# zalo/TetSim

Hardware: AMD Instinct MI355X
Metric: tet_solves_per_sec (higher is better)
Workload: dtype f32; 1 GPU; Kuhn-6 cube lattice 55x55x55 cells (998250 tets, 175616 particles), polar-decomposition Jacobi, 20 substeps/frame, dt=1/1200 s; solver=polar_jacobi, arithmetic=fast, formulation=reference (rest shape carried from substep to substep, 148 B/tet), tets=998250, particles=175616, parallelism=single GPU

## Files before the change

### tetsim_amd/csrc/pj_blocked.hip

```cpp
#define TETSIM_FAST 1
#include <cstdio>
#include <algorithm>
#include <cstdlib>
#include <type_traits>
#include <vector>

#include "collide.h"
#include "dev_common.h"
#include "dev_store.h"
#include "host_prep.h"
#include "pj_lab.h"

namespace tetsim {
namespace {

#include "pj_math.inc"
#include "pj_blocked_lab.inc"


__device__ __forceinline__ uint32_t xcd_tile(uint32_t b, uint32_t tiles_per_xcd) { return (b & 7u) * tiles_per_xcd + (b >> 3); }

struct VertexOut { f3 p, vel, pred; };
__device__ __forceinline__ VertexOut pjb_vertex_update(f3 acc, float wsum, f3 prev, const DevParams& P, uint32_t v) {
    const float rw = __builtin_amdgcn_rcpf(wsum);
    f3 p = F3(acc.x * rw, acc.y * rw, acc.z * rw);
    const bool grabbed = static_cast<int32_t>(v) == P.grab_local || static_cast<int32_t>(v) == P.grab_local2;
    if (grabbed) p = F3(P.grab[0], P.grab[1], P.grab[2]);
    p.x = fminf(fmaxf(p.x, P.lo[0]), P.hi[0]);
    p.y = fminf(fmaxf(p.y, P.lo[1]), P.hi[1]);
    p.z = fminf(fmaxf(p.z, P.lo[2]), P.hi[2]);
    if (p.y < 0.0f) {
        p.y = 0.0f;
        const float Fx = prev.x - p.x, Fz = prev.z - p.z;
        const float fr = fminf(1.0f, P.dt * P.friction);
        p.x = fmaf(Fx, fr, p.x);
        p.z = fmaf(Fz, fr, p.z);
    }
    if (P.n_colliders != 0u && !grabbed) collide_f32<true>(p.x, p.y, p.z, prev.x, prev.y, prev.z, P);
    const float dt = P.dt;
    const float rdt = __builtin_amdgcn_rcpf(dt);
    VertexOut o;
    o.p = p;
    const float gx = dt * 0.0f, gy = dt * P.gravity, gz = dt * 0.0f;
    o.vel = F3(fmaf(rdt, p.x - prev.x, gx), fmaf(rdt, p.y - prev.y, gy), fmaf(rdt, p.z - prev.z, gz));
    o.pred = F3(fmaf(dt, o.vel.x, p.x), fmaf(dt, o.vel.y, p.y), fmaf(dt, o.vel.z, p.z));
    return o;
}

constexpr uint32_t kTile = kBlockTile;

__device__ __forceinline__ f3 lean_fourth_corner(const f3 r[4]) {
    return F3(-((r[0].x + r[1].x) + r[2].x), -((r[0].y + r[1].y) + r[2].y), -((r[0].z + r[1].z) + r[2].z));
}
struct PJHaloWait { const PJPeerSync* w; const uint32_t* vflag; uint32_t* error; uint32_t timeout_ms; const float4* ghosts; };
constexpr int kModeCarried = 0, kModeConstantRest = 1, kModeLeanState = 2;
inline int blk_mode(const PJBlk& d) { return pjb_mode(d); }
struct PJPoll { uint32_t block, want; uint32_t* error; uint32_t timeout_ms; };
template <int kMode, bool kFused, bool kAlt = false, bool kHaloWait = false, bool kPoll = false>
__device__ __forceinline__ void pjb_tet_body(const PJBlk& d, uint32_t tile_first, uint32_t tile_count, uint32_t tiles_per_xcd TETSIM_DBG_PARAM,
                                             [[maybe_unused]] const PJHaloWait* hw = nullptr, const uint32_t stamp = 0u, [[maybe_unused]] const PJPoll* poll = nullptr) {
    __shared__ float4 s_pos[kTile];
    __shared__ float s_gx[4 * kTile];
    __shared__ float s_gy[4 * kTile];
    __shared__ float s_gz[4 * kTile];
    __shared__ uint2 s_ent[kTile];

    constexpr bool kLean = kMode == kModeConstantRest;
    uint32_t block_index = blockIdx.x;
    if constexpr (kPoll) block_index = poll->block;
    const uint32_t rel = xcd_tile(block_index, tiles_per_xcd);
    if (rel >= tile_count) return;
    const uint32_t b = tile_first + rel;
    const uint32_t tid = threadIdx.x;
    TETSIM_LAB_TILE_BEGIN();
    const uint32_t t0 = d.blk_tet_off[b], ntb = d.blk_tet_off[b + 1] - t0;
    const uint32_t v0 = d.blk_vert_off[b], nu = d.blk_vert_off[b + 1] - v0;

    const bool has_slot = tid < nu, has_tet = tid < ntb;
    const uint32_t slot = v0 + (has_slot ? tid : 0u), e = t0 + (has_tet ? tid : 0u);
    const uint32_t vid = static_cast<uint32_t>(d.blk_verts[slot]);
    const uint32_t range = has_slot ? d.lc_range[slot] : 0u;
    uint32_t src[8];
    uint32_t src8 = 0xffffffffu;
    [[maybe_unused]] uint32_t maxsrc = 0;
    if constexpr (kFused) {
        maxsrc = d.blk_maxsrc[b];
        const uint32_t* col = d.slot_src + slot;
#pragma unroll
        for (uint32_t j = 0; j < 8u; j++) src[j] = (j < maxsrc) ? col[static_cast<size_t>(j) * d.ns_pad] : 0xffffffffu;
        if (maxsrc > 8u) src8 = col[8ull * d.ns_pad];
    }
    const uchar4 li = d.tet_lidx[e];
    auto rec4 = [](const float4* a, uint32_t i) { if constexpr (kPoll) return load_coherent(a, i); else return a[i]; };
    float4 ra = make_float4(0.0f, 0.0f, 0.0f, 0.0f), rb = ra, rc = ra, q_old = make_float4(0.0f, 0.0f, 0.0f, 1.0f);
    auto load_record = [&]() {
        ra = rec4(d.rest_a, e); rb = rec4(d.rest_b, e);
        if constexpr (kMode == kModeLeanState) { if constexpr (kPoll) rc.x = load_coherent1(d.rest_c1, e); else rc.x = d.rest_c1[e]; }
        else { rc = rec4(d.rest_c, e); q_old = rec4(d.quat, e); }
    };
    bool record_late = false;
    if constexpr (kPoll) record_late = poll->want != 0u;
    if (!record_late) load_record();
    const float V = d.vol[e];
    const uint2 ent_row = d.lc_ent[e];
    float4 pos_stage;
    if constexpr (kFused) {
        f3 g[8];
#pragma unroll
        for (uint32_t j = 0; j < 8u; j++) {
            const float4 t = d.partial_prev[src[j] == 0xffffffffu ? 0u : src[j]];
            g[j] = src[j] == 0xffffffffu ? F3(0.0f, 0.0f, 0.0f) : xyz(t);
        }
        const float4 t8 = d.partial_prev[src8 == 0xffffffffu ? 0u : src8];
        const float4 prev4 = d.fin_in[vid];
        const float wsum = d.wsum[vid];
        f3 acc = F3(0.0f, 0.0f, 0.0f);
#pragma unroll
        for (uint32_t j = 0; j < 8u; j++) { acc.x += g[j].x; acc.y += g[j].y; acc.z += g[j].z; }
        if (src8 != 0xffffffffu) { acc.x += t8.x; acc.y += t8.y; acc.z += t8.z; }
        if (maxsrc > 9u) {
            const uint32_t* col = d.slot_src + slot;
            for (uint32_t j = 9u; j < maxsrc; j++) {
                const uint32_t sj = col[static_cast<size_t>(j) * d.ns_pad];
                const float4 tj = d.partial_prev[sj == 0xffffffffu ? 0u : sj];
                if (sj != 0xffffffffu) { acc.x += tj.x; acc.y += tj.y; acc.z += tj.z; }
            }
        }
        const VertexOut o = pjb_vertex_update(acc, wsum, xyz(prev4), *d.params, vid);
        pos_stage = make_float4(o.pred.x, o.pred.y, o.pred.z, 0.0f);
        if (has_slot && ((range >> 15) & 1u)) {
            store_wt(d.fin_out, vid, make_float4(o.p.x, o.p.y, o.p.z, 0.0f));
            if (d.vel) store_wt(d.vel, vid, make_float4(o.vel.x, o.vel.y, o.vel.z, 0.0f));
        }
    } else if constexpr (kHaloWait) {
        if (tid < 64u) {
            const PJPeerSync& w = *hw->w;
            const uint32_t* word = tid == 0u ? hw->vflag : (tid <= w.n_wait ? w.wait[tid - 1u] : nullptr);
            bool pending = word != nullptr;
            const long long t0 = wall_clock64(), limit = 100000ll * hw->timeout_ms;
            while (true) {
                if (pending) pending = __hip_atomic_load(word, __ATOMIC_RELAXED, __HIP_MEMORY_SCOPE_SYSTEM) == 0u;
                if (__builtin_amdgcn_ballot_w64(pending) == 0ull) break;
                __builtin_amdgcn_s_sleep(16);
                if (limit && wall_clock64() - t0 > limit) { if (tid == 0) __hip_atomic_store(hw->error, 1u, __ATOMIC_RELAXED, __HIP_MEMORY_SCOPE_SYSTEM); break; }
            }
            if (w.delay_us && w.n_wait) { const long long d0 = wall_clock64(); while (wall_clock64() - d0 < 100ll * w.delay_us) __builtin_amdgcn_s_sleep(8); }
        }
        __syncthreads();
        const bool ghost = vid >= d.nv_owned;
        const float4 own = load_coherent(d.pos_pred, ghost ? 0u : vid), gh = load_coherent(hw->ghosts, ghost ? vid - d.nv_owned : 0u);
        pos_stage = ghost ? gh : own;
    } else if constexpr (kAlt) {
        const uint32_t g = vid - d.nv_owned;
        const float4* src = vid >= d.nv_owned ? (g < d.n_ghost1 ? d.ghost_alt + g : d.ghost2 + (g - d.n_ghost1)) : d.pos_pred + vid;
        pos_stage = *src;
    } else if constexpr (kPoll) {
        pos_stage = load_coherent(d.pos_pred, vid);
        if (poll->want != 0u) {
            bool pend = has_slot && __float_as_uint(pos_stage.w) != poll->want;
            if (__builtin_amdgcn_ballot_w64(pend) != 0ull) {
                const long long t0 = wall_clock64(), limit = 100000ll * poll->timeout_ms;
                do {
                    __builtin_amdgcn_s_sleep(TETSIM_POLL_SLEEP);
                    asm volatile("" ::: "memory");
                    if (pend) { pos_stage = load_coherent(d.pos_pred, vid); pend = __float_as_uint(pos_stage.w) != poll->want; }
                    if (limit && pend && wall_clock64() - t0 > limit) { __hip_atomic_store(poll->error, 1u, __ATOMIC_RELAXED, __HIP_MEMORY_SCOPE_SYSTEM); pend = false; }
                } while (__builtin_amdgcn_ballot_w64(pend) != 0ull);
            }
            __syncthreads();
            load_record();
        }
    } else {
        pos_stage = d.pos_pred[vid];
    }
    if (has_slot) s_pos[tid] = pos_stage;
    if (has_tet) s_ent[tid] = ent_row;
    TETSIM_STAMP(1);
    __builtin_amdgcn_s_waitcnt(0x0F70);
    __syncthreads();
    TETSIM_STAMP(2);

    if (has_tet) {
        f3 cur[4], rest[4], goal[4];
        cur[0] = xyz(s_pos[li.x]); cur[1] = xyz(s_pos[li.y]); cur[2] = xyz(s_pos[li.z]); cur[3] = xyz(s_pos[li.w]);
        rest[0] = F3(ra.x, ra.y, ra.z); rest[1] = F3(ra.w, rb.x, rb.y);
        rest[2] = F3(rb.z, rb.w, rc.x); rest[3] = F3(rc.y, rc.z, rc.w);
        if constexpr (kMode == kModeLeanState) rest[3] = lean_fourth_corner(rest);
        float4 q_new;
        f3 cc;
        TETSIM_LAB_SOLVE_TET(cur, rest, q_old, q_new, goal, cc);
        TETSIM_STAMP(3);
        const f3 vcc = cc * V;
#pragma unroll
        for (int k = 0; k < 4; k++) {
            s_gx[k * kTile + tid] = fmaf(goal[k].x, V, vcc.x);
            s_gy[k * kTile + tid] = fmaf(goal[k].y, V, vcc.y);
            s_gz[k * kTile + tid] = fmaf(goal[k].z, V, vcc.z);
        }
        if constexpr (kMode != kModeLeanState) store_wt(d.quat, e, q_new);
        if (!kLean && TETSIM_DBG_STORE_REST) {
            store_wt(d.rest_a, e, make_float4(goal[0].x, goal[0].y, goal[0].z, goal[1].x));
            store_wt(d.rest_b, e, make_float4(goal[1].y, goal[1].z, goal[2].x, goal[2].y));
            if constexpr (kMode == kModeLeanState) store_wt1(d.rest_c1, e, goal[2].z);
            else store_wt(d.rest_c, e, make_float4(goal[2].z, goal[3].x, goal[3].y, goal[3].z));
        }
    }
    TETSIM_STAMP(4);
    if constexpr (kPoll) __builtin_amdgcn_s_waitcnt(0x0F70);
    __syncthreads();
    TETSIM_STAMP(5);

    if (tid < nu) {
        const uint32_t first = range & 0x7ffu, last = range >> 16;
        const uint16_t* ent = reinterpret_cast<const uint16_t*>(s_ent);
        auto plane = [](const float* base, uint32_t byte_off) { return *reinterpret_cast<const float*>(reinterpret_cast<const char*>(base) + byte_off); };
        float4 acc = make_float4(0.0f, 0.0f, 0.0f, 0.0f);
        uint32_t i = first;
        for (; i + 4u <= last; i += 4u) {
            uint32_t o[4];
            float gx[4], gy[4], gz[4];
#pragma unroll
            for (uint32_t j = 0; j < 4u; j++) o[j] = static_cast<uint32_t>(ent[i + j]) << 2;
#pragma unroll
            for (uint32_t j = 0; j < 4u; j++) { gx[j] = plane(s_gx, o[j]); gy[j] = plane(s_gy, o[j]); gz[j] = plane(s_gz, o[j]); }
#pragma unroll
            for (uint32_t j = 0; j < 4u; j++) { acc.x += gx[j]; acc.y += gy[j]; acc.z += gz[j]; }
        }
        for (; i < last; i++) {
            const uint32_t o = static_cast<uint32_t>(ent[i]) << 2;
            acc.x += plane(s_gx, o); acc.y += plane(s_gy, o); acc.z += plane(s_gz, o);
        }
        acc.w = __uint_as_float(stamp);
        store_wt(d.partial, v0 + tid, acc);
    }
    TETSIM_STAMP(6);
}

__global__ __launch_bounds__(kTile, 2) void pjb_tet_kernel(PJBlk d, uint32_t tile_first, uint32_t tile_count,
                                                        uint32_t tiles_per_xcd TETSIM_DBG_PARAM) {
    pjb_tet_body<kModeCarried, false>(d, tile_first, tile_count, tiles_per_xcd TETSIM_DBG_ARG);
}
__global__ __launch_bounds__(kTile, 2) void pjb_tet_kernel_constant_rest(PJBlk d, uint32_t tile_first, uint32_t tile_count,
                                                                      uint32_t tiles_per_xcd TETSIM_DBG_PARAM) {
    pjb_tet_body<kModeConstantRest, false>(d, tile_first, tile_count, tiles_per_xcd TETSIM_DBG_ARG);
}
__global__ __launch_bounds__(kTile, 2) void pjb_tet_kernel_lean(PJBlk d, uint32_t tile_first, uint32_t tile_count,
                                                             uint32_t tiles_per_xcd TETSIM_DBG_PARAM) {
    pjb_tet_body<kModeLeanState, false>(d, tile_first, tile_count, tiles_per_xcd TETSIM_DBG_ARG);
}
__device__ __forceinline__ void clear_then_raise(uint32_t* clear, uint32_t* sig) {
    if (blockIdx.x == 0 && threadIdx.x == 0) {
        if (clear) __hip_atomic_store(clear, 0u, __ATOMIC_RELAXED, __HIP_MEMORY_SCOPE_AGENT);
        if (sig) __hip_atomic_store(sig, 1u, __ATOMIC_RELEASE, __HIP_MEMORY_SCOPE_AGENT);
    }
}
struct TetRaise { uint32_t* sig; uint32_t* clear; };
struct TetAlt { uint32_t unused; };
struct TetHwait { PJPeerSync w; const uint32_t* vflag; uint32_t* error; uint32_t timeout_ms; const float4* ghosts; };
struct TetFused { uint32_t unused; };
template <int kMode, class Extra>
__global__ __launch_bounds__(kTile, 2) void pjb_tet_kernel_x(PJBlk d, uint32_t tile_first, uint32_t tile_count, uint32_t tiles_per_xcd, Extra x TETSIM_DBG_PARAM) {
    if constexpr (std::is_same_v<Extra, TetRaise>) {
        clear_then_raise(x.clear, x.sig);
        pjb_tet_body<kMode, false>(d, tile_first, tile_count, tiles_per_xcd TETSIM_DBG_ARG);
    } else if constexpr (std::is_same_v<Extra, TetAlt>) {
        pjb_tet_body<kMode, false, true>(d, tile_first, tile_count, tiles_per_xcd TETSIM_DBG_ARG);
    } else if constexpr (std::is_same_v<Extra, TetHwait>) {
        if (blockIdx.x == 0 && threadIdx.x < x.w.n_raise) __hip_atomic_store(x.w.raise[threadIdx.x], 1u, __ATOMIC_RELEASE, __HIP_MEMORY_SCOPE_SYSTEM);
        const PJHaloWait hw = {&x.w, x.vflag, x.error, x.timeout_ms, x.ghosts};
        pjb_tet_body<kMode, false, false, true>(d, tile_first, tile_count, tiles_per_xcd TETSIM_DBG_ARG, &hw);
    } else {
        pjb_tet_body<kMode, true>(d, tile_first, tile_count, tiles_per_xcd TETSIM_DBG_ARG);
    }
}
template <class Extra>
void launch_tet_x(hipStream_t s, const PJBlk& d, uint32_t tile_first, uint32_t tile_count, const Extra& x, hipEvent_t e0 = nullptr, hipEvent_t e1 = nullptr) {
    if (tile_count == 0) return;
    const uint32_t per_xcd = (tile_count + 7u) / 8u;
    const int mode = blk_mode(d);
    auto* kernel = mode == kModeConstantRest ? pjb_tet_kernel_x<kModeConstantRest, Extra> : mode == kModeLeanState ? pjb_tet_kernel_x<kModeLeanState, Extra> : pjb_tet_kernel_x<kModeCarried, Extra>;
    if (e0) hipExtLaunchKernelGGL(kernel, dim3(per_xcd * 8u), dim3(kTile), 0, s, e0, e1, 0, d, tile_first, tile_count, per_xcd, x TETSIM_DBG_LAUNCH);
    else hipLaunchKernelGGL(kernel, dim3(per_xcd * 8u), dim3(kTile), 0, s, d, tile_first, tile_count, per_xcd, x TETSIM_DBG_LAUNCH);
}

constexpr int kFrameIters = TETSIM_LAB_FRAME_ITERS;
template <int kMode, bool kLocal>
__device__ __forceinline__ void pjb_frame_body(const PJBlk& d, const DevParams& P, const uint32_t n, const int32_t* const block_tile, float4* const pbuf0, float4* const pbuf1,
                                               uint32_t* const err, const uint32_t timeout_ms) {
    __shared__ float4 s_pos[kTile];
    __shared__ float s_gx[4 * kTile];
    __shared__ float s_gy[4 * kTile];
    __shared__ float s_gz[4 * kTile];
    __shared__ uint2 s_ent[kTile];

    constexpr bool kLean = kMode == kModeConstantRest;
    const int32_t bt = block_tile[blockIdx.x];
    if (bt < 0) return;
    const uint32_t b = static_cast<uint32_t>(bt);
    const uint32_t tid = threadIdx.x;
    TETSIM_LAB_FRAME_BEGIN();
    const uint32_t t0 = d.blk_tet_off[b], ntb = d.blk_tet_off[b + 1] - t0;
    const uint32_t v0 = d.blk_vert_off[b], nu = d.blk_vert_off[b + 1] - v0;
    const bool has_slot = tid < nu, has_tet = tid < ntb;
    const uint32_t slot = v0 + (has_slot ? tid : 0u), e = t0 + (has_tet ? tid : 0u);
    const uint32_t vid = static_cast<uint32_t>(d.blk_verts[slot]);
    const uint32_t range = has_slot ? d.lc_range[slot] : 0u;
    const uint32_t maxsrc = d.blk_maxsrc[b];
    uint32_t src[9];
    {
        const uint32_t* col = d.slot_src + slot;
#pragma unroll
        for (uint32_t j = 0; j < 9u; j++) src[j] = (has_slot && j < maxsrc) ? col[static_cast<size_t>(j) * d.ns_pad] : 0xffffffffu;
    }
    const uchar4 li = d.tet_lidx[e];
    const float4 ra = d.rest_a[e], rb = d.rest_b[e];
    float4 rc = make_float4(0.0f, 0.0f, 0.0f, 0.0f), q = make_float4(0.0f, 0.0f, 0.0f, 1.0f);
    if constexpr (kMode == kModeLeanState) rc.x = d.rest_c1[e];
    else { rc = d.rest_c[e]; q = d.quat[e]; }
    const float V = d.vol[e];
    s_ent[tid] = has_tet ? d.lc_ent[e] : make_uint2(0u, 0u);
    f3 rest[4];
    rest[0] = F3(ra.x, ra.y, ra.z); rest[1] = F3(ra.w, rb.x, rb.y);
    rest[2] = F3(rb.z, rb.w, rc.x); rest[3] = F3(rc.y, rc.z, rc.w);
    f3 prev = xyz(d.pos_final[vid]);
    const float wsum = d.wsum[vid];
    f3 stage = xyz(d.pos_pred[vid]);
    const uint32_t epoch = d.epoch ? d.epoch : P.epoch;
    const uint32_t first = range & 0x7ffu, last = range >> 16;
    const bool owner = has_slot && ((range >> 15) & 1u);
    float4* const pbuf[2] = {pbuf0, pbuf1};
    const long long limit = 100000ll * timeout_ms;

    auto gather_update = [&](const uint32_t s) -> VertexOut {
        const float4* buf = pbuf[s & 1u];
        const uint32_t expect = epoch + s;
        f3 g[9];
        uint32_t pend = 0;
#pragma unroll
        for (uint32_t j = 0; j < 9u; j++) { g[j] = F3(0.0f, 0.0f, 0.0f); pend |= (src[j] != 0xffffffffu ? 1u : 0u) << j; }
        const long long w0 = limit ? wall_clock64() : 0ll;
        while (__builtin_amdgcn_ballot_w64(pend != 0u) != 0ull) {
            float4 t[9];
#pragma unroll
            for (uint32_t j = 0; j < 9u; j++)
                if ((pend >> j) & 1u) t[j] = kLocal ? load_l2(buf, src[j]) : load_coherent(buf, src[j]);
            FRAME_POLL();
#pragma unroll
            for (uint32_t j = 0; j < 9u; j++)
                if (((pend >> j) & 1u) && __float_as_uint(t[j].w) == expect) { g[j] = xyz(t[j]); pend &= ~(1u << j); }
            if (limit && pend != 0u && wall_clock64() - w0 > limit) {
                __hip_atomic_store(err, 1u, __ATOMIC_RELAXED, __HIP_MEMORY_SCOPE_SYSTEM);
                pend = 0u;
            }
        }
        f3 acc = F3(0.0f, 0.0f, 0.0f);
#pragma unroll
        for (uint32_t j = 0; j < 8u; j++) { acc.x += g[j].x; acc.y += g[j].y; acc.z += g[j].z; }
        if (src[8] != 0xffffffffu) { acc.x += g[8].x; acc.y += g[8].y; acc.z += g[8].z; }
        if (maxsrc > 9u) {
            const uint32_t* col = d.slot_src + slot;
            for (uint32_t j = 9u; j < maxsrc; j++) {
                const uint32_t sj = has_slot ? col[static_cast<size_t>(j) * d.ns_pad] : 0xffffffffu;
                bool miss = sj != 0xffffffffu;
                f3 gj = F3(0.0f, 0.0f, 0.0f);
                while (__builtin_amdgcn_ballot_w64(miss) != 0ull) {
                    if (miss) {
                        const float4 t = kLocal ? load_l2(buf, sj) : load_coherent(buf, sj);
                        if (__float_as_uint(t.w) == expect) { gj = xyz(t); miss = false; }
                    }
                    if (limit && miss && wall_clock64() - w0 > limit) {
                        __hip_atomic_store(err, 1u, __ATOMIC_RELAXED, __HIP_MEMORY_SCOPE_SYSTEM);
                        miss = false;
                    }
                }
                acc.x += gj.x; acc.y += gj.y; acc.z += gj.z;
            }
        }
        return pjb_vertex_update(acc, wsum, prev, P, vid);
    };

    for (uint32_t s = 0; s < n; s++) {
        FRAME_STAMP(0);
        if (s > 0u) {
            const VertexOut o = gather_update(s - 1u);
            prev = o.p;
            stage = o.pred;
        }
        FRAME_STAMP(1);
        if (has_slot) s_pos[tid] = make_float4(stage.x, stage.y, stage.z, 0.0f);
        __syncthreads();
        FRAME_STAMP(2);
        if (has_tet) {
            f3 cur[4], r[4], goal[4];
            cur[0] = xyz(s_pos[li.x]); cur[1] = xyz(s_pos[li.y]); cur[2] = xyz(s_pos[li.z]); cur[3] = xyz(s_pos[li.w]);
#pragma unroll
            for (int k = 0; k < 4; k++) r[k] = rest[k];
            if constexpr (kMode == kModeLeanState) r[3] = lean_fourth_corner(rest);
            float4 q_new;
            f3 cc;
            pj_solve_tet(cur, r, q, q_new, goal, kFrameIters, true, kLean, !kLean, &cc, d.rot_exit_w2);
            if constexpr (kMode != kModeLeanState) q = q_new;
            if (!kLean) {
#pragma unroll
                for (int k = 0; k < 4; k++) rest[k] = goal[k];
            }
            const f3 vcc = cc * V;
#pragma unroll
            for (int k = 0; k < 4; k++) {
                s_gx[k * kTile + tid] = fmaf(goal[k].x, V, vcc.x);
                s_gy[k * kTile + tid] = fmaf(goal[k].y, V, vcc.y);
                s_gz[k * kTile + tid] = fmaf(goal[k].z, V, vcc.z);
            }
        }
        FRAME_STAMP(3);
        __syncthreads();
        FRAME_STAMP(4);
        if (has_slot) {
            const uint16_t* ent = reinterpret_cast<const uint16_t*>(s_ent);
            auto plane = [](const float* base, uint32_t byte_off) { return *reinterpret_cast<const float*>(reinterpret_cast<const char*>(base) + byte_off); };
            float4 acc = make_float4(0.0f, 0.0f, 0.0f, 0.0f);
            uint32_t i = first;
            for (; i + 4u <= last; i += 4u) {
                uint32_t o[4];
                float gx[4], gy[4], gz[4];
#pragma unroll
                for (uint32_t j = 0; j < 4u; j++) o[j] = static_cast<uint32_t>(ent[i + j]) << 2;
#pragma unroll
                for (uint32_t j = 0; j < 4u; j++) { gx[j] = plane(s_gx, o[j]); gy[j] = plane(s_gy, o[j]); gz[j] = plane(s_gz, o[j]); }
#pragma unroll
                for (uint32_t j = 0; j < 4u; j++) { acc.x += gx[j]; acc.y += gy[j]; acc.z += gz[j]; }
            }
            for (; i < last; i++) {
                const uint32_t o = static_cast<uint32_t>(ent[i]) << 2;
                acc.x += plane(s_gx, o); acc.y += plane(s_gy, o); acc.z += plane(s_gz, o);
            }
            acc.w = __uint_as_float(epoch + s);
            if constexpr (kLocal) store_plain(pbuf[s & 1u], v0 + tid, acc);
            else store_wt(pbuf[s & 1u], v0 + tid, acc);
        }
        FRAME_STAMP(5);
    }
    const VertexOut o = gather_update(n - 1u);
    TETSIM_LAB_FRAME_END();
    if (owner) {
        store_wt(d.pos_final, vid, make_float4(o.p.x, o.p.y, o.p.z, 0.0f));
        store_wt(d.vel, vid, make_float4(o.vel.x, o.vel.y, o.vel.z, 0.0f));
        store_wt(d.pos_pred, vid, make_float4(o.pred.x, o.pred.y, o.pred.z, 0.0f));
    }
    if (has_tet) {
        if constexpr (kMode != kModeLeanState) store_wt(d.quat, e, q);
        if (!kLean) {
            store_wt(d.rest_a, e, make_float4(rest[0].x, rest[0].y, rest[0].z, rest[1].x));
            store_wt(d.rest_b, e, make_float4(rest[1].y, rest[1].z, rest[2].x, rest[2].y));
            if constexpr (kMode == kModeLeanState) store_wt1(d.rest_c1, e, rest[2].z);
            else store_wt(d.rest_c, e, make_float4(rest[2].z, rest[3].x, rest[3].y, rest[3].z));
        }
    }
}
#define TETSIM_FRAME_KERNEL(name, mode, local)                                                                                         \
    __global__ __launch_bounds__(kTile, 2) void name(PJBlk d, uint32_t n, const int32_t* block_tile, float4* pbuf0, float4* pbuf1, uint32_t* err, \
                                                     uint32_t timeout_ms, DevParams pv, DevParams* pdev) {                             \
        if (blockIdx.x == 0u && threadIdx.x == 0u) store_params(pdev, pv);              \
        pjb_frame_body<mode, local>(d, pv, n, block_tile, pbuf0, pbuf1, err, timeout_ms);                                              \
    }
TETSIM_FRAME_KERNEL(pjb_frame_kernel, kModeCarried, false)
TETSIM_FRAME_KERNEL(pjb_frame_kernel_constant_rest, kModeConstantRest, false)
TETSIM_FRAME_KERNEL(pjb_frame_kernel_lean, kModeLeanState, false)
TETSIM_FRAME_KERNEL(pjb_frame_kernel_local, kModeCarried, true)
TETSIM_FRAME_KERNEL(pjb_frame_kernel_constant_rest_local, kModeConstantRest, true)
TETSIM_FRAME_KERNEL(pjb_frame_kernel_lean_local, kModeLeanState, true)
#undef TETSIM_FRAME_KERNEL
__global__ void pjb_probe_xcd_kernel(uint32_t* out) {
    if (threadIdx.x == 0) out[blockIdx.x] = __builtin_amdgcn_s_getreg(20 | (0 << 6) | (3 << 11));
}

__device__ __forceinline__ void await_done(const PJSync& y) {
    if (threadIdx.x == 0) {
        const long long t0 = wall_clock64(), limit = 100000ll * y.timeout_ms;
        while (__hip_atomic_load(y.flag, __ATOMIC_ACQUIRE, __HIP_MEMORY_SCOPE_AGENT) == 0u) {
            __builtin_amdgcn_s_sleep(4);
            if (limit && wall_clock64() - t0 > limit) {
                __hip_atomic_store(y.error, 1u, __ATOMIC_RELAXED, __HIP_MEMORY_SCOPE_SYSTEM);
                return;
            }
        }
        __hip_atomic_store(y.flag, 0u, __ATOMIC_RELAXED, __HIP_MEMORY_SCOPE_AGENT);
    }
}

template <bool kPeer = false, bool kCoherent = false>
__device__ __forceinline__ void pjb_vertex_body(const PJBlk& d, uint32_t first, uint32_t count, const PJPeer* peer = nullptr) {
    const uint32_t i = blockIdx.x * 64u + threadIdx.x;
    if (i >= count) return;
    const uint32_t v = first + i;

    float4 acc = make_float4(0.0f, 0.0f, 0.0f, 0.0f);
    const uint32_t* col = d.vp_ell + v;
    for (uint32_t j0 = 0; j0 < d.vp_cols; j0 += 8u) {
        uint32_t idx[8];
        float4 g[8];
#pragma unroll
        for (uint32_t j = 0; j < 8u; j++) idx[j] = (j0 + j < d.vp_cols) ? col[static_cast<size_t>(j0 + j) * d.nv_pad] : 0xffffffffu;
#pragma unroll
        for (uint32_t j = 0; j < 8u; j++) {
            if constexpr (kCoherent) { const float4 t = load_coherent(d.partial, idx[j] != 0xffffffffu ? idx[j] : 0u); g[j] = idx[j] != 0xffffffffu ? t : make_float4(0.0f, 0.0f, 0.0f, 0.0f); }
            else g[j] = idx[j] != 0xffffffffu ? d.partial[idx[j]] : make_float4(0.0f, 0.0f, 0.0f, 0.0f);
        }
#pragma unroll
        for (uint32_t j = 0; j < 8u; j++) { acc.x += g[j].x; acc.y += g[j].y; acc.z += g[j].z; }
        if (__all(idx[7] == 0xffffffffu)) break;
    }
    const VertexOut o = pjb_vertex_update(xyz(acc), d.wsum[v], xyz(d.fin_in[v]), *d.params, v);
    store_wt(d.fin_out, v, make_float4(o.p.x, o.p.y, o.p.z, 0.0f));
    if (d.vel) store_wt(d.vel, v, make_float4(o.vel.x, o.vel.y, o.vel.z, 0.0f));
    store_wt(d.pos_pred, v, make_float4(o.pred.x, o.pred.y, o.pred.z, 0.0f));
    if constexpr (kPeer) {
        const float4 pred4 = make_float4(o.pred.x, o.pred.y, o.pred.z, 0.0f), fin4 = make_float4(o.p.x, o.p.y, o.p.z, 0.0f);
        const uint32_t* col = peer->slots + v;
        for (uint32_t c = 0; c < peer->cols; c++) {
            const uint32_t e = col[static_cast<size_t>(c) * peer->stride];
            for (uint32_t k = 0; k < peer->n; k++) {
                if (peer->ghost[k] && e != 0xffffffffu && (e >> 24) == k) store_wt(peer->ghost[k], e & 0xffffffu, pred4);
                if (peer->fin[k] && e != 0xffffffffu && (e >> 24) == k) store_wt(peer->fin[k], e & 0xffffffu, fin4);
            }
        }
        if (peer->slots2) {
            const uint32_t* col2 = peer->slots2 + v;
            for (uint32_t c = 0; c < peer->cols2; c++) {
                const uint32_t e = col2[static_cast<size_t>(c) * peer->stride];
                for (uint32_t k = 0; k < peer->n; k++)
                    if (peer->ghost2[k] && e != 0xffffffffu && (e >> 24) == k) store_wt(peer->ghost2[k], e & 0xffffffu, pred4);
            }
        }
    }
}

__global__ __launch_bounds__(64) void pjb_vertex_kernel(PJBlk d, uint32_t first, uint32_t count) { pjb_vertex_body(d, first, count); }

template <int kMode>
__global__ __launch_bounds__(kTile, 2) void pjb_call_kernel(PJBlk d, uint32_t n_sub, uint32_t tile_count, uint32_t tiles_per_xcd, uint32_t tet_blocks, uint32_t blocks_per_sub,
                                                           uint32_t* err, uint32_t timeout_ms, DevParams pv, DevParams* pdev TETSIM_DBG_PARAM) {
    const uint32_t sub = blockIdx.x / blocks_per_sub, r = blockIdx.x - sub * blocks_per_sub;
    const uint32_t stamp = (d.epoch ? d.epoch : pv.epoch) + sub + 1u;
    if (blockIdx.x == 0u && threadIdx.x == 0u) store_params(pdev, pv);
    if (r < tet_blocks) {
        const PJPoll poll = {r, sub ? stamp - 1u : 0u, err, timeout_ms};
        pjb_tet_body<kMode, false, false, false, true>(d, 0u, tile_count, tiles_per_xcd TETSIM_DBG_ARG, nullptr, stamp, &poll);
        return;
    }
    const uint32_t v = (r - tet_blocks) * kTile + threadIdx.x;
    if (v >= d.nv_owned) return;
    float4 acc = make_float4(0.0f, 0.0f, 0.0f, 0.0f);
    const uint32_t* col = d.vp_ell + v;
    const long long limit = 100000ll * timeout_ms;
    const float wsum = d.wsum[v];
    float4 prev = load_coherent(d.fin_in, v);
    for (uint32_t j0 = 0; j0 < d.vp_cols; j0 += 8u) {
        uint32_t idx[8];
        float4 g[8];
#pragma unroll
        for (uint32_t j = 0; j < 8u; j++) idx[j] = (j0 + j < d.vp_cols) ? col[static_cast<size_t>(j0 + j) * d.nv_pad] : 0xffffffffu;
        uint32_t pend = 0;
#pragma unroll
        for (uint32_t j = 0; j < 8u; j++) {
            const float4 t = load_coherent(d.partial, idx[j] != 0xffffffffu ? idx[j] : 0u);
            g[j] = idx[j] != 0xffffffffu ? t : make_float4(0.0f, 0.0f, 0.0f, 0.0f);
            pend |= (idx[j] != 0xffffffffu && __float_as_uint(t.w) != stamp ? 1u : 0u) << j;
        }
        if (__builtin_amdgcn_ballot_w64(pend != 0u) != 0ull) {
            const long long t0 = wall_clock64();
            do {
                __builtin_amdgcn_s_sleep(TETSIM_POLL_SLEEP);
                asm volatile("" ::: "memory");
#pragma unroll
                for (uint32_t j = 0; j < 8u; j++)
                    if ((pend >> j) & 1u) {
                        const float4 t = load_coherent(d.partial, idx[j]);
                        if (__float_as_uint(t.w) == stamp) { g[j] = t; pend &= ~(1u << j); }
                    }
                if (limit && pend != 0u && wall_clock64() - t0 > limit) {
                    __hip_atomic_store(err, 1u, __ATOMIC_RELAXED, __HIP_MEMORY_SCOPE_SYSTEM);
                    pend = 0u;
                }
            } while (__builtin_amdgcn_ballot_w64(pend != 0u) != 0ull);
        }
#pragma unroll
        for (uint32_t j = 0; j < 8u; j++) { acc.x += g[j].x; acc.y += g[j].y; acc.z += g[j].z; }
        if (__all(idx[7] == 0xffffffffu)) break;
    }
    if (sub) {
        const long long t0 = wall_clock64();
        while (__float_as_uint(prev.w) != stamp - 1u) {
            __builtin_amdgcn_s_sleep(4);
            asm volatile("" ::: "memory");
            prev = load_coherent(d.fin_in, v);
            if (limit && wall_clock64() - t0 > limit) { __hip_atomic_store(err, 1u, __ATOMIC_RELAXED, __HIP_MEMORY_SCOPE_SYSTEM); break; }
        }
    }
    const VertexOut o = pjb_vertex_update(xyz(acc), wsum, xyz(prev), pv, v);
    store_wt(d.fin_out, v, make_float4(o.p.x, o.p.y, o.p.z, __uint_as_float(stamp)));
    if (d.vel && sub + 1u == n_sub) store_wt(d.vel, v, make_float4(o.vel.x, o.vel.y, o.vel.z, 0.0f));
    store_wt(d.pos_pred, v, make_float4(o.pred.x, o.pred.y, o.pred.z, __uint_as_float(stamp)));
}
__global__ __launch_bounds__(64) void pjb_vertex_kernel_raise(PJBlk d, uint32_t first, uint32_t count, uint32_t* sig, uint32_t* clear) {
    clear_then_raise(clear, sig);
    pjb_vertex_body(d, first, count);
}
__global__ __launch_bounds__(64) void pjb_vertex_kernel_await(PJBlk d, uint32_t first, uint32_t count, uint32_t* flag, uint32_t* error, uint32_t timeout_ms) {
    if (threadIdx.x == 0) {
        const long long t0 = wall_clock64(), limit = 100000ll * timeout_ms;
        while (__hip_atomic_load(flag, __ATOMIC_RELAXED, __HIP_MEMORY_SCOPE_AGENT) == 0u) {
            __builtin_amdgcn_s_sleep(16);
            if (limit && wall_clock64() - t0 > limit) { __hip_atomic_store(error, 1u, __ATOMIC_RELAXED, __HIP_MEMORY_SCOPE_SYSTEM); break; }
        }
    }
    __builtin_amdgcn_wave_barrier();
    pjb_vertex_body<false, true>(d, first, count);
}
__global__ __launch_bounds__(64) void pjb_vertex_kernel_peer(PJBlk d, uint32_t first, uint32_t count, PJPeer peer, uint32_t* sig, PJClear clr) {
    if (blockIdx.x == 0 && threadIdx.x == 0) {
        for (uint32_t i = 0; i < clr.n; i++) __hip_atomic_store(clr.word[i], 0u, __ATOMIC_RELAXED, __HIP_MEMORY_SCOPE_SYSTEM);
        if (sig) __hip_atomic_store(sig, 1u, __ATOMIC_RELEASE, __HIP_MEMORY_SCOPE_AGENT);
    }
    pjb_vertex_body<true>(d, first, count, &peer);
}
__global__ void pjb_wait_peers_kernel(uint32_t* flag, uint32_t* error, uint32_t timeout_ms, PJPeerSync w) {
    PJSync y;
    y.flag = flag; y.error = error; y.timeout_ms = timeout_ms;
    const uint32_t t = threadIdx.x;
    if (t < w.n_raise) __hip_atomic_store(w.raise[t], 1u, __ATOMIC_RELEASE, __HIP_MEMORY_SCOPE_SYSTEM);
    if (y.flag) await_done(y);
    if (t < w.n_wait) {
        const long long t0 = wall_clock64(), limit = 100000ll * y.timeout_ms;
        while (__hip_atomic_load(w.wait[t], __ATOMIC_ACQUIRE, __HIP_MEMORY_SCOPE_SYSTEM) == 0u) {
            __builtin_amdgcn_s_sleep(4);
            if (limit && wall_clock64() - t0 > limit) { __hip_atomic_store(y.error, 1u, __ATOMIC_RELAXED, __HIP_MEMORY_SCOPE_SYSTEM); break; }
        }
        __hip_atomic_store(w.wait[t], 0u, __ATOMIC_RELAXED, __HIP_MEMORY_SCOPE_SYSTEM);
        if (w.delay_us) { const long long d0 = wall_clock64(); while (wall_clock64() - d0 < 100ll * w.delay_us) __builtin_amdgcn_s_sleep(8); }
    }
}
__global__ void pjb_wait_kernel(uint32_t* flag, uint32_t* error, uint32_t timeout_ms) {
    PJSync y;
    y.flag = flag; y.error = error; y.timeout_ms = timeout_ms;
    await_done(y);
}
__global__ void pjb_signal_kernel(uint32_t* flag, uint32_t* clear) {
    if (threadIdx.x == 0) {
        if (clear) __hip_atomic_store(clear, 0u, __ATOMIC_RELAXED, __HIP_MEMORY_SCOPE_AGENT);
        __hip_atomic_store(flag, 1u, __ATOMIC_RELEASE, __HIP_MEMORY_SCOPE_AGENT);
    }
}

__global__ __launch_bounds__(256) void pjb_recover_quat_kernel(const float4* __restrict__ r0a, const float4* __restrict__ r0b, const float4* __restrict__ r0c,
                                                              const float4* __restrict__ ca, const float4* __restrict__ cb, const float* __restrict__ cc1,
                                                              float4* __restrict__ quat, uint32_t nt) {
    const uint32_t e = blockIdx.x * 256u + threadIdx.x;
    if (e >= nt) return;
    const float4 a0 = r0a[e], b0 = r0b[e], c0 = r0c[e], a = ca[e], b = cb[e];
    const float c1 = cc1[e];
    const float4 qp = quat[e];
    const double s[3][3] = {{a0.x, a0.y, a0.z}, {a0.w, b0.x, b0.y}, {b0.z, b0.w, c0.x}};
    const double c[3][3] = {{a.x, a.y, a.z}, {a.w, b.x, b.y}, {b.z, b.w, c1}};
    auto cr = [](const double* u, const double* v, double* o) { o[0] = u[1] * v[2] - u[2] * v[1]; o[1] = u[2] * v[0] - u[0] * v[2]; o[2] = u[0] * v[1] - u[1] * v[0]; };
    double inv[3][3];
    cr(s[1], s[2], inv[0]); cr(s[2], s[0], inv[1]); cr(s[0], s[1], inv[2]);
    const double det = s[0][0] * inv[0][0] + s[0][1] * inv[0][1] + s[0][2] * inv[0][2];
    if (!(fabs(det) > 1.0e-300)) return;
    const double rd = 1.0 / det;
    double R[3][3];
    for (int i = 0; i < 3; i++)
        for (int j = 0; j < 3; j++) R[i][j] = (c[0][i] * inv[0][j] + c[1][i] * inv[1][j] + c[2][i] * inv[2][j]) * rd;
    const double tr = R[0][0] + R[1][1] + R[2][2];
    double x, y, z, w;
    if (tr > 0.0) { w = tr + 1.0; x = R[2][1] - R[1][2]; y = R[0][2] - R[2][0]; z = R[1][0] - R[0][1]; }
    else if (R[0][0] >= R[1][1] && R[0][0] >= R[2][2]) { x = 1.0 + R[0][0] - R[1][1] - R[2][2]; y = R[0][1] + R[1][0]; z = R[0][2] + R[2][0]; w = R[2][1] - R[1][2]; }
    else if (R[1][1] >= R[2][2]) { y = 1.0 + R[1][1] - R[0][0] - R[2][2]; x = R[0][1] + R[1][0]; z = R[1][2] + R[2][1]; w = R[0][2] - R[2][0]; }
    else { z = 1.0 + R[2][2] - R[0][0] - R[1][1]; x = R[0][2] + R[2][0]; y = R[1][2] + R[2][1]; w = R[1][0] - R[0][1]; }
    const double n2 = x * x + y * y + z * z + w * w;
    if (!(n2 > 0.0) || !(n2 < 1.0e300)) return;
    double k = 1.0 / sqrt(n2);
    if (x * qp.x + y * qp.y + z * qp.z + w * qp.w < 0.0) k = -k;
    quat[e] = make_float4(static_cast<float>(x * k), static_cast<float>(y * k), static_cast<float>(z * k), static_cast<float>(w * k));
}

__global__ __launch_bounds__(256) void pjb_repredict_kernel(PJBlk d) {
    const uint32_t v = blockIdx.x * 256u + threadIdx.x;
    if (v >= d.nv_owned) return;
    const f3 pred = xyz(d.pos_final[v]) + xyz(d.vel[v]) * d.params->dt;
    d.pos_pred[v] = make_float4(pred.x, pred.y, pred.z, 0.0f);
}

}

void pjb_launch_tet(hipStream_t s, const PJBlk& d, uint32_t tile_first, uint32_t tile_count, hipEvent_t e0, hipEvent_t e1, uint32_t* raise_word,
                    uint32_t* clear_word) {
    if (tile_count == 0) return;
    if (raise_word || clear_word) return launch_tet_x(s, d, tile_first, tile_count, TetRaise{raise_word, clear_word}, e0, e1);
    const uint32_t per_xcd = (tile_count + 7u) / 8u;
    const int mode = blk_mode(d);
    auto* kernel = mode == kModeConstantRest ? pjb_tet_kernel_constant_rest : mode == kModeLeanState ? pjb_tet_kernel_lean : pjb_tet_kernel;
    if (e0) hipExtLaunchKernelGGL(kernel, dim3(per_xcd * 8u), dim3(kTile), 0, s, e0, e1, 0, d, tile_first, tile_count, per_xcd TETSIM_DBG_LAUNCH);
    else hipLaunchKernelGGL(kernel, dim3(per_xcd * 8u), dim3(kTile), 0, s, d, tile_first, tile_count, per_xcd TETSIM_DBG_LAUNCH);
}
void pjb_launch_call(hipStream_t s, const PJBlk& d, uint32_t n, uint32_t* err, uint32_t timeout_ms, const DevParams& params, DevParams* params_dev) {
    if (d.nb == 0 || n == 0) return;
    const uint32_t per_xcd = (d.nb + 7u) / 8u, tet_blocks = per_xcd * 8u, per_sub = pjb_call_blocks_per_sub(d.nb, d.nv_owned, kTile);
    const int mode = blk_mode(d);
    auto* kernel = mode == kModeConstantRest ? pjb_call_kernel<kModeConstantRest> : mode == kModeLeanState ? pjb_call_kernel<kModeLeanState> : pjb_call_kernel<kModeCarried>;
    hipLaunchKernelGGL(kernel, dim3(per_sub * n), dim3(kTile), 0, s, d, n, d.nb, per_xcd, tet_blocks, per_sub, err, timeout_ms, params, params_dev TETSIM_DBG_LAUNCH);
}
void pjb_launch_tet_fused(hipStream_t s, const PJBlk& d, hipEvent_t e0, hipEvent_t e1) { launch_tet_x(s, d, 0u, d.nb, TetFused{0u}, e0, e1); }
void pjb_launch_frame(hipStream_t s, const PJBlk& d, uint32_t n, const int32_t* block_tile, uint32_t blocks, bool local, float4* pbuf0, float4* pbuf1,
                      uint32_t* err, uint32_t timeout_ms, const DevParams& params, DevParams* params_dev, hipEvent_t e0, hipEvent_t e1) {
    if (d.nb == 0 || n == 0 || blocks == 0) return;
    const int mode = blk_mode(d);
    auto* kernel = local ? (mode == kModeConstantRest ? pjb_frame_kernel_constant_rest_local : mode == kModeLeanState ? pjb_frame_kernel_lean_local : pjb_frame_kernel_local)
                         : (mode == kModeConstantRest ? pjb_frame_kernel_constant_rest : mode == kModeLeanState ? pjb_frame_kernel_lean : pjb_frame_kernel);
    if (e0) hipExtLaunchKernelGGL(kernel, dim3(blocks), dim3(kTile), 0, s, e0, e1, 0, d, n, block_tile, pbuf0, pbuf1, err, timeout_ms, params, params_dev);
    else hipLaunchKernelGGL(kernel, dim3(blocks), dim3(kTile), 0, s, d, n, block_tile, pbuf0, pbuf1, err, timeout_ms, params, params_dev);
}
uint32_t pjb_frame_capacity(int mode, uint32_t* compute_units) {
    int per_cu = 0, dev = 0;
    hipDeviceProp_t prop;
    if (hipGetDevice(&dev) != hipSuccess || hipGetDeviceProperties(&prop, dev) != hipSuccess) return 0;
    int per_cu_any = 0;
    auto* k_local = mode == kModeConstantRest ? pjb_frame_kernel_constant_rest_local : mode == kModeLeanState ? pjb_frame_kernel_lean_local : pjb_frame_kernel_local;
    auto* k_any = mode == kModeConstantRest ? pjb_frame_kernel_constant_rest : mode == kModeLeanState ? pjb_frame_kernel_lean : pjb_frame_kernel;
    const hipError_t e = hipOccupancyMaxActiveBlocksPerMultiprocessor(&per_cu, k_local, static_cast<int>(kTile), 0);
    const hipError_t e2 = hipOccupancyMaxActiveBlocksPerMultiprocessor(&per_cu_any, k_any, static_cast<int>(kTile), 0);
    if (e != hipSuccess || e2 != hipSuccess || per_cu <= 0 || per_cu_any <= 0) return 0;
    per_cu = std::min(per_cu, per_cu_any);
    if (compute_units) *compute_units = static_cast<uint32_t>(prop.multiProcessorCount);
    return static_cast<uint32_t>(per_cu);
}
void pjb_wait_capacity(int mode, uint32_t* vertex_waves, uint32_t* hwait_blocks) {
    *vertex_waves = 0; *hwait_blocks = 0;
    int per_cu_v = 0, per_cu_t = 0, dev = 0;
    hipDeviceProp_t prop;
    if (hipGetDevice(&dev) != hipSuccess || hipGetDeviceProperties(&prop, dev) != hipSuccess) return;
    if (hipOccupancyMaxActiveBlocksPerMultiprocessor(&per_cu_v, pjb_vertex_kernel_await, 64, 0) != hipSuccess) per_cu_v = 0;
    auto* k_hwait = mode == kModeConstantRest ? pjb_tet_kernel_x<kModeConstantRest, TetHwait> : mode == kModeLeanState ? pjb_tet_kernel_x<kModeLeanState, TetHwait> : pjb_tet_kernel_x<kModeCarried, TetHwait>;
    const hipError_t e = hipOccupancyMaxActiveBlocksPerMultiprocessor(&per_cu_t, k_hwait, static_cast<int>(kTile), 0);
    if (e != hipSuccess) per_cu_t = 0;
    const uint32_t cus = static_cast<uint32_t>(std::max(prop.multiProcessorCount, 0));
    *vertex_waves = static_cast<uint32_t>(std::max(per_cu_v, 0)) * cus / 2u;
    *hwait_blocks = static_cast<uint32_t>(std::max(per_cu_t, 0)) * cus / 4u;
}
uint32_t pjb_probe_xcd(hipStream_t s, uint32_t blocks) {
    uint32_t* d_out = nullptr;
    if (blocks < 16u || hipMalloc(reinterpret_cast<void**>(&d_out), blocks * sizeof(uint32_t)) != hipSuccess) return 0;
    std::vector<uint32_t> out(blocks, 0xffffffffu);
    hipLaunchKernelGGL(pjb_probe_xcd_kernel, dim3(blocks), dim3(64), 0, s, d_out);
    const bool ok = hipStreamSynchronize(s) == hipSuccess && hipMemcpy(out.data(), d_out, blocks * sizeof(uint32_t), hipMemcpyDeviceToHost) == hipSuccess;
    (void)hipFree(d_out);
    if (!ok) return 0;
    for (uint32_t i = 0; i < 8u; i++)
        for (uint32_t j = 0; j < i; j++) if (out[i] == out[j]) return 0;
    for (uint32_t i = 8u; i < blocks; i++) if (out[i] != out[i & 7u]) return 0;
    return 8;
}
void pjb_launch_wait_peers(hipStream_t s, const PJSync& y, const PJPeerSync& w) { hipLaunchKernelGGL(pjb_wait_peers_kernel, dim3(1), dim3(64), 0, s, y.flag, y.error, y.timeout_ms, w); }
void pjb_launch_vertex_peer(hipStream_t s, const PJBlk& d, uint32_t first, uint32_t count, const PJPeer& peer, uint32_t* raise_word, const PJClear& clr) {
    if (count == 0) return;
    hipLaunchKernelGGL(pjb_vertex_kernel_peer, dim3((count + 63u) / 64u), dim3(64), 0, s, d, first, count, peer, raise_word, clr);
}
void pjb_launch_tet_hwait(hipStream_t s, const PJBlk& d, uint32_t tile_first, uint32_t tile_count, const PJSync& yv, const PJPeerSync& w, const float4* ghosts) {
    launch_tet_x(s, d, tile_first, tile_count, TetHwait{w, yv.flag, yv.error, yv.timeout_ms, ghosts});
}
void pjb_launch_tet_alt(hipStream_t s, const PJBlk& d, uint32_t tile_first, uint32_t tile_count) { launch_tet_x(s, d, tile_first, tile_count, TetAlt{0u}); }
void pjb_launch_wait(hipStream_t s, const PJSync& y) { hipLaunchKernelGGL(pjb_wait_kernel, dim3(1), dim3(64), 0, s, y.flag, y.error, y.timeout_ms); }
void pjb_launch_signal(hipStream_t s, const PJSync& y, uint32_t* clear_word) { hipLaunchKernelGGL(pjb_signal_kernel, dim3(1), dim3(64), 0, s, y.flag, clear_word); }
void pjb_launch_vertex_await(hipStream_t s, const PJBlk& d, uint32_t first, uint32_t count, const PJSync& y, hipEvent_t e0, hipEvent_t e1) {
    if (count == 0) return;
    if (e0) hipExtLaunchKernelGGL(pjb_vertex_kernel_await, dim3((count + 63u) / 64u), dim3(64), 0, s, e0, e1, 0, d, first, count, y.flag, y.error, y.timeout_ms);
    else hipLaunchKernelGGL(pjb_vertex_kernel_await, dim3((count + 63u) / 64u), dim3(64), 0, s, d, first, count, y.flag, y.error, y.timeout_ms);
}
void pjb_launch_vertex(hipStream_t s, const PJBlk& d, uint32_t first, uint32_t count, hipEvent_t e0, hipEvent_t e1, uint32_t* raise_word, uint32_t* clear_word) {
    if (count == 0) return;
    if (raise_word || clear_word) {
        if (e0) hipExtLaunchKernelGGL(pjb_vertex_kernel_raise, dim3((count + 63u) / 64u), dim3(64), 0, s, e0, e1, 0, d, first, count, raise_word, clear_word);
        else hipLaunchKernelGGL(pjb_vertex_kernel_raise, dim3((count + 63u) / 64u), dim3(64), 0, s, d, first, count, raise_word, clear_word);
        return;
    }
    if (e0) hipExtLaunchKernelGGL(pjb_vertex_kernel, dim3((count + 63u) / 64u), dim3(64), 0, s, e0, e1, 0, d, first, count);
    else hipLaunchKernelGGL(pjb_vertex_kernel, dim3((count + 63u) / 64u), dim3(64), 0, s, d, first, count);
}
void pjb_launch_recover_quats(hipStream_t s, const PJBlk& d, const float4* rest0_a, const float4* rest0_b, const float4* rest0_c) {
    if (d.nt == 0 || !d.lean_state) return;
    hipLaunchKernelGGL(pjb_recover_quat_kernel, dim3((d.nt + 255u) / 256u), dim3(256), 0, s, rest0_a, rest0_b, rest0_c, d.rest_a, d.rest_b, d.rest_c1, d.quat, d.nt);
}
void pjb_launch_repredict(hipStream_t s, const PJBlk& d) {
    if (d.nv_owned == 0) return;
    hipLaunchKernelGGL(pjb_repredict_kernel, dim3((d.nv_owned + 255u) / 256u), dim3(256), 0, s, d);
}

}
```

### tetsim_amd/csrc/pj_lab.h

```cpp
#pragma once

#define TETSIM_ROTATION_ITERATIONS 9

#ifndef TETSIM_ABLATION
#define TETSIM_DBG_PARAM
#define TETSIM_DBG_ARG
#define TETSIM_DBG_LAUNCH
#define TETSIM_DBG_STORE_REST true
#define TETSIM_LAB_FRAME_ITERS TETSIM_ROTATION_ITERATIONS
#define TETSIM_W2LOG_PARAM
#define TETSIM_W2LOG(i, v) do { } while (0)
#define TETSIM_LAB_TILE_BEGIN() do { } while (0)
#define TETSIM_STAMP(i) do { } while (0)
#define TETSIM_LAB_SOLVE_TET(cur, rest, q_old, q_new, goal, cc) \
    pj_solve_tet(cur, rest, q_old, q_new, goal, TETSIM_ROTATION_ITERATIONS, true, kLean, !kLean, &cc, d.rot_exit_w2)
#define TETSIM_LAB_FRAME_BEGIN() do { } while (0)
#define FRAME_STAMP(i) do { } while (0)
#define FRAME_POLL() do { } while (0)
#define TETSIM_LAB_FRAME_END() do { } while (0)
#else
#define TETSIM_DBG_PARAM , uint32_t dbg
#define TETSIM_DBG_ARG , dbg
#define TETSIM_DBG_LAUNCH , tet_mode()
#define TETSIM_DBG_STORE_REST (!(dbg & 16u))
#define TETSIM_LAB_FRAME_ITERS 9
#define TETSIM_W2LOG_PARAM , float* w2log = nullptr
#define TETSIM_W2LOG(i, v) do { if (w2log) w2log[(i)] = (v); } while (0)
#define TETSIM_STAMP(i) do { if (d.trace && tid == 0) d.trace[8ull * b + (i)] = __builtin_amdgcn_s_memtime(); } while (0)
#define TETSIM_LAB_TILE_BEGIN() do {                                                                                              \
        if (d.trace && tid == 0) d.trace[8ull * b + 7] = __builtin_amdgcn_s_getreg((4 << 0) | (0 << 6) | (31 << 11));  \
        TETSIM_STAMP(0);                                                                                                           \
        if (const uint32_t st_ = (dbg >> 8) & 0xffu; st_ != 0u && blockIdx.x < 2048u) {                                            \
            const uint32_t k_ = (dbg & 0x10000u) ? (blockIdx.x >> 3) & 7u : (blockIdx.x >> 8) & 7u;                                \
            for (uint32_t i_ = 0; i_ < k_ * st_; i_++) __builtin_amdgcn_s_sleep(1);                                                \
        }                                                                                                                          \
    } while (0)
#define TETSIM_LAB_SOLVE_TET(cur, rest, q_old, q_new, goal, cc) do {                                                              \
        float w2log_[9];                                                                                                           \
        for (int i_ = 0; i_ < 9; i_++) w2log_[i_] = -1.0f;             \
        pj_solve_tet(cur, rest, q_old, q_new, goal, static_cast<int>(dbg & 15u), !(dbg & 64u), kLean, !kLean, &cc, d.rot_exit_w2,   \
                     d.iter_hist ? w2log_ : nullptr);                                                                              \
        if (d.iter_hist) pjb_log_iterations(d.iter_hist, w2log_);                                                                  \
    } while (0)
#define TETSIM_LAB_FRAME_BEGIN() unsigned long long fr_acc[5] = {0, 0, 0, 0, 0}, fr_last = 0, fr_polls = 0
#define FRAME_STAMP(i) do { if (d.trace && tid == 0) { const unsigned long long now_ = __builtin_amdgcn_s_memtime(); if ((i) > 0) fr_acc[(i) > 0 ? (i) - 1 : 0] += now_ - fr_last; fr_last = now_; } } while (0)
#define FRAME_POLL() do { if (tid == 0) fr_polls++; } while (0)
#define TETSIM_LAB_FRAME_END() do {                                                                                                \
        if (d.trace && tid == 0) {                                                                                                 \
            for (int i_ = 0; i_ < 5; i_++) d.trace[8ull * b + i_] = fr_acc[i_];                                                    \
            d.trace[8ull * b + 5] = fr_polls; d.trace[8ull * b + 6] = n;                                                           \
            d.trace[8ull * b + 7] = __builtin_amdgcn_s_getreg(20 | (0 << 6) | (3 << 11));                              \
        }                                                                                                                          \
    } while (0)
#endif
```

Before: 34240 M tet-solves/s.

## Gate late record load on block's own partial release flag instead of block barrier

In the polling path, each block first spins on its own partial-sum release flag at v0 using a wave-uniform readfirstlane check. Once that flag arrives it loads the rest-shape record early, before polling the neighbour positions. This removes the __syncthreads plus record load that previously came after the per-vertex position poll, so the record fetch overlaps with waiting on neighbours. It adds an extra coherent load and a second spin loop, and it relies on the own-partial flag implying that the record is ready.

```diff
diff --git a/tetsim_amd/csrc/pj_blocked.hip b/tetsim_amd/csrc/pj_blocked.hip
--- a/tetsim_amd/csrc/pj_blocked.hip
+++ b/tetsim_amd/csrc/pj_blocked.hip
@@ -91,6 +91,9 @@
         if (maxsrc > 8u) src8 = col[8ull * d.ns_pad];
     }
     const uchar4 li = d.tet_lidx[e];
+    constexpr bool kOwnRelease = kPoll && !TETSIM_CALL_RECORD_LATE;
+    [[maybe_unused]] float4 own_sum = make_float4(0.0f, 0.0f, 0.0f, 0.0f);
+    if constexpr (kOwnRelease) own_sum = load_coherent(d.partial, nu ? v0 : 0u);
     auto rec4 = [](const float4* a, uint32_t i) { if constexpr (kPoll) return load_coherent(a, i); else return a[i]; };
     float4 ra = make_float4(0.0f, 0.0f, 0.0f, 0.0f), rb = ra, rc = ra, q_old = make_float4(0.0f, 0.0f, 0.0f, 1.0f);
     auto load_record = [&]() {
@@ -155,6 +158,25 @@
         const float4* src = vid >= d.nv_owned ? (g < d.n_ghost1 ? d.ghost_alt + g : d.ghost2 + (g - d.n_ghost1)) : d.pos_pred + vid;
         pos_stage = *src;
     } else if constexpr (kPoll) {
+        if constexpr (kOwnRelease) {
+            if (record_late) {
+                uint32_t seen = __builtin_amdgcn_readfirstlane(__float_as_uint(own_sum.w));
+                if (nu != 0u && seen != poll->want) {
+                    const long long t0 = wall_clock64(), limit = 100000ll * poll->timeout_ms;
+                    do {
+                        __builtin_amdgcn_s_sleep(TETSIM_POLL_SLEEP);
+                        asm volatile("" ::: "memory");
+                        seen = __builtin_amdgcn_readfirstlane(__float_as_uint(load_coherent(d.partial, v0).w));
+                        if (limit && seen != poll->want && wall_clock64() - t0 > limit) {
+                            __hip_atomic_store(poll->error, 1u, __ATOMIC_RELAXED, __HIP_MEMORY_SCOPE_SYSTEM);
+                            break;
+                        }
+                    } while (seen != poll->want);
+                }
+                load_record();
+                TETSIM_STAMP_RELEASED();
+            }
+        }
         pos_stage = load_coherent(d.pos_pred, vid);
         if (poll->want != 0u) {
             bool pend = has_slot && __float_as_uint(pos_stage.w) != poll->want;
@@ -167,8 +189,11 @@
                     if (limit && pend && wall_clock64() - t0 > limit) { __hip_atomic_store(poll->error, 1u, __ATOMIC_RELAXED, __HIP_MEMORY_SCOPE_SYSTEM); pend = false; }
                 } while (__builtin_amdgcn_ballot_w64(pend) != 0ull);
             }
-            __syncthreads();
-            load_record();
+            if constexpr (!kOwnRelease) {
+                __syncthreads();
+                load_record();
+                TETSIM_STAMP_RELEASED();
+            }
         }
     } else {
         pos_stage = d.pos_pred[vid];
diff --git a/tetsim_amd/csrc/pj_lab.h b/tetsim_amd/csrc/pj_lab.h
--- a/tetsim_amd/csrc/pj_lab.h
+++ b/tetsim_amd/csrc/pj_lab.h
@@ -1,6 +1,10 @@
 #pragma once
 
 #define TETSIM_ROTATION_ITERATIONS 9
+
+#ifndef TETSIM_CALL_RECORD_LATE
+#define TETSIM_CALL_RECORD_LATE 0
+#endif
 
 #ifndef TETSIM_ABLATION
 #define TETSIM_DBG_PARAM
@@ -12,6 +16,7 @@
 #define TETSIM_W2LOG(i, v) do { } while (0)
 #define TETSIM_LAB_TILE_BEGIN() do { } while (0)
 #define TETSIM_STAMP(i) do { } while (0)
+#define TETSIM_STAMP_RELEASED() do { } while (0)
 #define TETSIM_LAB_SOLVE_TET(cur, rest, q_old, q_new, goal, cc) \
     pj_solve_tet(cur, rest, q_old, q_new, goal, TETSIM_ROTATION_ITERATIONS, true, kLean, !kLean, &cc, d.rot_exit_w2)
 #define TETSIM_LAB_FRAME_BEGIN() do { } while (0)
@@ -27,6 +32,7 @@
 #define TETSIM_W2LOG_PARAM , float* w2log = nullptr
 #define TETSIM_W2LOG(i, v) do { if (w2log) w2log[(i)] = (v); } while (0)
 #define TETSIM_STAMP(i) do { if (d.trace && tid == 0) d.trace[8ull * b + (i)] = __builtin_amdgcn_s_memtime(); } while (0)
+#define TETSIM_STAMP_RELEASED() TETSIM_STAMP(7)
 #define TETSIM_LAB_TILE_BEGIN() do {                                                                                              \
         if (d.trace && tid == 0) d.trace[8ull * b + 7] = __builtin_amdgcn_s_getreg((4 << 0) | (0 << 6) | (31 << 11));  \
         TETSIM_STAMP(0);                                                                                                           \
```

After: 33700 M tet-solves/s. 1.6% lower.
